# tky823/DNN-based_source_separation

Measured on AMD Instinct MI355X. Metric: separated audio frames/sec (fwd+bwd), Conv-TasNet 2-spk 4s@8kHz, higher is better.
Workload: dtype f32 (f16x3: fp32 operands/accumulators, products from a 2-part fp16 split on the fp16 MFMA; fp32-MFMA pass beside it); 1 GPU; Conv-TasNet paper-best (N=512,L=16,B=128,H=512,Sc=128,P=3,X=8,R=3) 2-spk, 4 s @ 8 kHz synthetic mixtures, 16 utterances/GPU, fwd + PIT(NegSI-SDR) + bwd + clip(5) + Adam; global_batch=16, per_gpu_batch=16, parallelism=dp1, rccl_ranks=0, launch=recorded sequence, one sep_run_sequence call per step

## Files before the change

dnn-based_source_separation_amd/csrc/gemm_coop.hip:

```cpp
#include "gemm_common.hpp"
#include <stddef.h>
#include <stdlib.h>
#include <type_traits>


namespace {

#ifndef COOP_PIPE
#define COOP_PIPE true
#endif
constexpr int CBN = 64;
constexpr int RBI = 264;
constexpr int COMAXK = 512;

template <int MI, int NS, bool AUX>
struct __attribute__((aligned(16))) CoopSmem {
    double red[8];
    float Bs[NS][4 * RBI];
    float Cs[AUX ? NS : 1][AUX ? 4 * RBI : 4];
    float Bp[2][CBN * 16];
    int be[2][CBN];
    float sc[COMAXK];
    float sh[AUX ? 4 : COMAXK];
    float epi_pad[(4 * EPI_WAVE_FLOATS > NS * 4 * RBI + (AUX ? NS * 4 * RBI : 4) + 2 * CBN * 16 + 2 * CBN + COMAXK + (AUX ? 4 : COMAXK))
                      ? 4 * EPI_WAVE_FLOATS - (NS * 4 * RBI + (AUX ? NS * 4 * RBI : 4) + 2 * CBN * 16 + 2 * CBN + COMAXK + (AUX ? 4 : COMAXK)) : 4];
};

template <int MI, int NS, bool BWD>
constexpr int coop_occupancy() {
    constexpr int by_lds = (int)((160 * 1024) / ((sizeof(CoopSmem<MI, NS, BWD>) + 511) / 512 * 512));
    constexpr int by_regs = MI == 4 ? 2 : MI == 2 ? 3 : 4;
    return by_lds < by_regs ? by_lds : by_regs;
}

__device__ __forceinline__ float co_vmax(const float a, const float b) {
    float r;
    asm("v_max_f32 %0, %1, %2" : "=v"(r) : "v"(a), "v"(b));
    return r;
}
__device__ __forceinline__ float co_quad_max(const float m) {
    float r, t;
    asm("s_nop 1\n\tv_max_f32_dpp %0, %1, %1 quad_perm:[1,0,3,2] row_mask:0xf bank_mask:0xf" : "=&v"(t) : "v"(m));
    asm("s_nop 1\n\tv_max_f32_dpp %0, %1, %1 quad_perm:[2,3,0,1] row_mask:0xf bank_mask:0xf" : "=&v"(r) : "v"(t));
    return r;
}
__device__ __forceinline__ void co_split2_pair(const float x0, const float x1, unsigned& hi, unsigned& lo) {
    const fp16x2_t h = __builtin_amdgcn_cvt_pkrtz(x0, x1);
    hi = __builtin_bit_cast(unsigned, h);
    float l0, l1;
    asm("v_fma_mix_f32 %0, %1, 1.0, -%2 op_sel_hi:[0,0,1]" : "=v"(l0) : "v"(x0), "v"(hi));
    asm("v_fma_mix_f32 %0, %1, 1.0, -%2 op_sel:[0,0,1] op_sel_hi:[0,0,1]" : "=v"(l1) : "v"(x1), "v"(hi));
    lo = __builtin_bit_cast(unsigned, __builtin_amdgcn_cvt_pkrtz(l0, l1));
}
template <int N, int I = 0, class F>
__device__ __forceinline__ void pco_unroll(F&& f) {
    if constexpr (I < N) { f(std::integral_constant<int, I>{}); pco_unroll<N, I + 1>(f); }
}
__device__ __forceinline__ f32x16 mfma_f16(const u32x4_t a, const u32x4_t b, const f32x16 c) {
    return __builtin_amdgcn_mfma_f32_32x32x16_f16(__builtin_bit_cast(f16x8_t, a), __builtin_bit_cast(f16x8_t, b), c, 0, 0, 0);
}
__device__ __forceinline__ float quad_max(float x) {
    x = fmaxf(x, __builtin_bit_cast(float, __builtin_amdgcn_update_dpp(0, __builtin_bit_cast(int, x), 0xB1, 0xF, 0xF, true)));
    x = fmaxf(x, __builtin_bit_cast(float, __builtin_amdgcn_update_dpp(0, __builtin_bit_cast(int, x), 0x4E, 0xF, 0xF, true)));
    return x;
}
template <int N>
__device__ __forceinline__ void wait_vm_lgkm0_barrier() {
    asm volatile("" ::: "memory");
    __builtin_amdgcn_s_waitcnt(0x0070 | (N & 15) | ((N >> 4) << 14));
    __builtin_amdgcn_s_barrier();
    asm volatile("" ::: "memory");
}

template <int MI, int PRO, bool SPLIT, int EF, int NS>
__global__ __launch_bounds__(256, (coop_occupancy<MI, NS, PRO == SEP_PRO_GLN_BWD>()))
void pw_gemm_coop_kernel(const sep_gemm_desc d) {
    constexpr bool P_PRELU = PRO == SEP_PRO_PRELU || PRO == SEP_PRO_GLN_PRELU;
    constexpr bool P_GLN = PRO == SEP_PRO_GLN || PRO == SEP_PRO_GLN_PRELU;
    constexpr bool P_BWD = PRO == SEP_PRO_GLN_BWD;
    constexpr int RW = 32 * MI;
    constexpr int BMc = 4 * RW;
    __shared__ CoopSmem<MI, NS, P_BWD> sm;
    using CoSmem = CoopSmem<MI, NS, P_BWD>;
    static_assert(sizeof(CoSmem) - offsetof(CoSmem, Bs) >= 4 * EPI_WAVE_FLOATS * sizeof(float), "epilogue transpose buffer");
    const int tid = threadIdx.x, lane = tid & 63;
    const int wid = __builtin_amdgcn_readfirstlane(tid >> 6);
    const int lk = lane >> 5, l31 = lane & 31;

    const int NR = d.M / BMc;
    const int ntile_t = d.ldt / CBN;
    const int NC = d.B * ntile_t;
    const int bid = blockIdx.x;
    const int xcd = bid & 7, jj = bid >> 3;
    const int rt = jj % NR;
    const int ct = (jj / NR) * 8 + xcd;
    if (ct >= NC) return;
    const int b = ct / ntile_t;
    const int t0 = (ct % ntile_t) * CBN;
    const int m0 = rt * BMc;
    const int nk = d.K / DK;
    const bool dead_tile = !P_BWD && t0 >= d.T;

    float alpha_p = 0.f, mu = 0.f, rstd = 1.f, mg = 0.f, mgx = 0.f;
    if (P_PRELU || P_BWD) alpha_p = d.pro_alpha[0];
    if (P_GLN || P_BWD) {
        gln_mu_rstd(d.pro_stats + (size_t)b * SEP_STATS_SLOTS * 2, d.count, d.eps, mu, rstd);
        for (int k = tid; k < d.K; k += 256) {
            if (P_BWD) sm.sc[k] = d.pro_gamma[k];
            else {
                const float scv = d.pro_gamma[k] * rstd;
                sm.sc[k] = scv;
                sm.sh[k] = d.pro_beta[k] - mu * scv;
            }
        }
    }
    if (P_BWD) {
        if (d.pro_bacc) gln_bwd_means(d.pro_bacc + (size_t)b * SEP_STATS_SLOTS * 2, d.pro_stats + (size_t)b * SEP_STATS_SLOTS * 2, d.count, d.eps, mg, mgx);
        else { mg = d.pro_bsum[2 * b]; mgx = d.pro_bsum[2 * b + 1]; }
    }
    float dalpha_pro = 0.f;
    asm volatile("" :: "v"(alpha_p), "v"(mu), "v"(rstd), "v"(mg), "v"(mgx));

    const int Ks1 = SPLIT ? d.k_split : d.K;
    const int split_chunk = SPLIT ? d.k_split / DK : -1;
    const size_t stepX = (size_t)DK * d.ldt;
    const unsigned offX = 4u * (unsigned)((lane >> 4) * d.ldt + 4 * (lane & 15));
    const float* baseX = d.X + ((size_t)b * Ks1 + 4 * wid) * d.ldt + t0;
    const float* baseC = P_BWD ? d.pro_aux + ((size_t)b * Ks1 + 4 * wid) * d.ldt + t0 : nullptr;
    int xi = 0, xst = 0;
    auto issue_x = [&]() {
        if (SPLIT && xi == split_chunk) baseX = d.X2 + ((size_t)b * (d.K - d.k_split) + 4 * wid) * d.ldt + t0;
        glds16_asm_once(baseX, offX, lds_addr(&sm.Bs[xst][wid * RBI]));
        if (P_BWD) glds16_asm_once(baseC, offX, lds_addr(&sm.Cs[P_BWD ? xst : 0][wid * RBI]));
        baseX += stepX;
        if (P_BWD) baseC += stepX;
        ++xi;
        xst = xst + 1 == NS ? 0 : xst + 1;
    };
    const char* Apk = reinterpret_cast<const char*>(d.A_pk) + (size_t)((m0 + wid * RW) >> 5) * nk * 2048;
    const unsigned a_lane = 16u * (unsigned)lane;

    f32x16 acc[MI][2];
#pragma unroll
    for (int mi = 0; mi < MI; ++mi)
#pragma unroll
        for (int ni = 0; ni < 2; ++ni)
#pragma unroll
            for (int r = 0; r < 16; ++r) acc[mi][ni][r] = 0.f;

    const int fsw = (l31 >> 2) & 3;
    const int c_hi = l31 * 16 + 4 * ((2 * lk) ^ fsw);
    const int c_lo = l31 * 16 + 4 * ((2 * lk + 1) ^ fsw);
    int bcur[2] = {0, 0};

    const int kq = lane & 3;
    const int col_s = 16 * wid + (lane >> 2);
    const int s_raw = kq * RBI + col_s;
    const int s_fsw = (col_s >> 2) & 3;
    const int s_hi = col_s * 16 + 4 * ((2 * (kq >> 1)) ^ s_fsw) + 2 * (kq & 1);
    const int s_lo = col_s * 16 + 4 * ((2 * (kq >> 1) + 1) ^ s_fsw) + 2 * (kq & 1);
    const bool s_live = t0 + col_s < d.T;
    const unsigned st_lane_off = 4u * (unsigned)(4 * kq * d.ldt + col_s);
    constexpr int UNSET = 10000;
    int bexp = UNSET;
    const bool fast_prelu = alpha_p >= 0.f && alpha_p <= 1.f;

    float raw[4], aux[4], v[4];
    float4 sc4 = make_float4(0.f, 0.f, 0.f, 0.f), sh4 = sc4;
    auto read_raw = [&](const int stage, const int kn) {
        const float* Bb = sm.Bs[stage];
#pragma unroll
        for (int j = 0; j < 4; ++j) raw[j] = Bb[s_raw + j * 64];
        if (P_BWD) {
            const float* Cb = sm.Cs[P_BWD ? stage : 0];
#pragma unroll
            for (int j = 0; j < 4; ++j) aux[j] = Cb[s_raw + j * 64];
        }
        if (P_GLN || P_BWD) sc4 = ld4(&sm.sc[kn * DK + 4 * kq]);
        if (P_GLN) sh4 = ld4(&sm.sh[kn * DK + 4 * kq]);
    };
    auto pro_vals = [&](const int kn) {
        const float scv[4] = {sc4.x, sc4.y, sc4.z, sc4.w};
        const float shv[4] = {sh4.x, sh4.y, sh4.z, sh4.w};
#pragma unroll
        for (int j = 0; j < 4; ++j) {
            float x = raw[j];
            if (P_BWD) {
                const float a = aux[j];
                const float u = prelu_f(a, alpha_p);
                const float xh = (u - mu) * rstd;
                const float du = rstd * (scv[j] * x - mg - xh * mgx);
                const float da = s_live ? du * prelu_grad(a, alpha_p) : 0.f;
                if (rt == 0) {
                    if (s_live && a <= 0.f) dalpha_pro += du * a;
                    float* srow = d.pro_store + ((size_t)b * d.K + kn * DK + j) * d.ldt + t0;
                    *reinterpret_cast<float*>(reinterpret_cast<char*>(srow) + (size_t)st_lane_off) = da;
                }
                x = da;
            } else {
                if (P_PRELU) x = fast_prelu ? co_vmax(x, alpha_p * x) : prelu_f(x, alpha_p);
                if (P_GLN) x = fmaf(x, scv[j], shv[j]);
            }
            v[j] = x;
        }
    };
    auto scale_vals = [&]() {
        float m = fmaxf(fmaxf(fabsf(v[0]), fabsf(v[1])), fmaxf(fabsf(v[2]), fabsf(v[3])));
        m = co_quad_max(m);
        const int e = __builtin_amdgcn_frexp_expf(m);
        const int e2 = __builtin_bit_cast(int, m) == 0 ? -3 * UNSET : e;
        bexp = e2 + bexp > 14 ? 9 - e : bexp;
    };
    unsigned h01, l01, h23, l23;
    auto split_vals = [&]() {
#pragma unroll
        for (int j = 0; j < 4; ++j) v[j] = __builtin_ldexpf(v[j], bexp);
        co_split2_pair(v[0], v[1], h01, l01);
        co_split2_pair(v[2], v[3], h23, l23);
    };
    auto write_vals = [&](const int pb) {
        float* Bp = sm.Bp[pb];
        *reinterpret_cast<uint2*>(Bp + s_hi) = make_uint2(h01, h23);
        *reinterpret_cast<uint2*>(Bp + s_lo) = make_uint2(l01, l23);
        sm.be[pb][col_s] = bexp;
    };

    u32x4_t pa[2][MI][2], pbv[2][2];
    int en[2];
    auto load_a = [&](auto setc, const int chunk) {
        constexpr int q = decltype(setc)::value;
#pragma unroll
        for (int mi = 0; mi < MI; ++mi) {
            const char* src = Apk + ((size_t)mi * nk + chunk) * 2048;
            pa[q][mi][0] = *reinterpret_cast<const u32x4_t*>(src + a_lane);
            pa[q][mi][1] = *reinterpret_cast<const u32x4_t*>(src + 1024 + a_lane);
        }
    };
    auto read_b = [&](const int pb) {
        const float* Bp = sm.Bp[pb];
#pragma unroll
        for (int ni = 0; ni < 2; ++ni) {
            pbv[ni][0] = *reinterpret_cast<const u32x4_t*>(Bp + ni * 32 * 16 + c_hi);
            pbv[ni][1] = *reinterpret_cast<const u32x4_t*>(Bp + ni * 32 * 16 + c_lo);
            en[ni] = sm.be[pb][ni * 32 + l31];
        }
    };
    auto rescale = [&]() {
#pragma unroll
        for (int ni = 0; ni < 2; ++ni) {
            const int delta = en[ni] - bcur[ni];
            if (__builtin_amdgcn_ballot_w64(delta != 0) != 0) {
#pragma unroll
                for (int mi = 0; mi < MI; ++mi)
#pragma unroll
                    for (int r = 0; r < 16; ++r) acc[mi][ni][r] = __builtin_ldexpf(acc[mi][ni][r], delta);
            }
            bcur[ni] = en[ni];
        }
    };
    constexpr int NM = 6 * MI;
    auto M = [&](auto setc, auto ic) {
        constexpr int q = decltype(setc)::value, i = decltype(ic)::value;
        constexpr int part = i / (2 * MI), mi = (i % (2 * MI)) / 2, ni = i % 2;
        constexpr int asel = part == 1 ? 1 : 0, bsel = part == 0 ? 1 : 0;
        acc[mi][ni] = mfma_f16(pa[q][mi][asel], pbv[ni][bsel], acc[mi][ni]);
        __builtin_amdgcn_sched_barrier(0);
    };
#define CO_I(k) std::integral_constant<int, (k)>{}
#define CO_SB() __builtin_amdgcn_sched_barrier(0)
    constexpr int GX = P_BWD ? 2 : 1;
    constexpr int KEEP = P_BWD ? 0 : (NS - 2) * GX + 2 * MI;
    static_assert(KEEP < 64, "vmcnt field");
    auto step = [&](auto pc, const int s) {
        constexpr int P = decltype(pc)::value;
        const bool more = s + 1 < nk;
        read_b(s & 1);
        if (more) {
            read_raw((s + 1) % NS, s + 1);
            load_a(CO_I(P ^ 1), s + 1);
        }
        CO_SB();
        rescale();
        CO_SB();
        pco_unroll<NM / 3>([&](auto ic) { M(CO_I(P), ic); });
        if (more) pro_vals(s + 1);
        CO_SB();
        pco_unroll<NM / 6>([&](auto ic) { M(CO_I(P), CO_I(decltype(ic)::value + NM / 3)); });
        if (more) scale_vals();
        CO_SB();
        pco_unroll<NM / 6>([&](auto ic) { M(CO_I(P), CO_I(decltype(ic)::value + NM / 2)); });
        if (more) split_vals();
        CO_SB();
        pco_unroll<NM / 6>([&](auto ic) { M(CO_I(P), CO_I(decltype(ic)::value + 2 * NM / 3)); });
        if (more) write_vals((s + 1) & 1);
        CO_SB();
        pco_unroll<NM / 6>([&](auto ic) { M(CO_I(P), CO_I(decltype(ic)::value + 5 * NM / 6)); });
        if (more) {
            if (KEEP > 0 && s + NS < nk) wait_vm_lgkm0_barrier<KEEP>();
            else wait_vm_lgkm0_barrier<0>();
            if (xi < nk) issue_x();
        }
    };

    if (!dead_tile) {
        __syncthreads();
        issue_x();
#pragma unroll
        for (int g = 0; g < NS - 1; ++g)
            if (xi < nk) issue_x();
        load_a(CO_I(0), 0);
        wait_vm_lgkm0_barrier<0>();
        read_raw(0, 0);
        pro_vals(0);
        scale_vals();
        split_vals();
        write_vals(0);
        wait_vm_lgkm0_barrier<0>();
        if (xi < nk) issue_x();
        int s = 0;
        for (; s + 1 < nk; s += 2) {
            step(CO_I(0), s);
            step(CO_I(1), s + 1);
        }
        if (s < nk) step(CO_I(0), s);
#pragma unroll
        for (int mi = 0; mi < MI; ++mi)
#pragma unroll
            for (int ni = 0; ni < 2; ++ni)
#pragma unroll
                for (int r = 0; r < 16; ++r) acc[mi][ni][r] = __builtin_ldexpf(acc[mi][ni][r], -bcur[ni]);
    }
    __syncthreads();
    int etid = tid, eb = b, em0 = m0, et0 = t0;
    asm volatile("" : "+v"(etid), "+s"(eb), "+s"(em0), "+s"(et0));
    const int ewid = __builtin_amdgcn_readfirstlane(etid >> 6);
    const int elane = etid & 63;
    gemm_epilogue<EF, MI, true, 4, COOP_PIPE>(d, acc, eb, em0, et0, ewid, 0, elane >> 5, elane & 31, etid, &sm.Bs[0][0], sm.red, CBN);
    if (P_BWD && rt == 0) {
        const double sdal = block_sum_256<double>((double)dalpha_pro, sm.red);
        if (tid == 0) atomicAdd(d.pro_dalpha, sdal);
    }
}

constexpr int PMAXSEG = 64;
struct PackArgs {
    sep_pack_seg seg[PMAXSEG];
    int blk_start[PMAXSEG + 1];
    int nseg;
};

__global__ __launch_bounds__(256) void pack_weights_kernel(const PackArgs a) {
    int sgi = 0;
    while (sgi + 1 < a.nseg && (int)blockIdx.x >= a.blk_start[sgi + 1]) ++sgi;
    const sep_pack_seg sg = a.seg[sgi];
    const int lane = threadIdx.x & 63;
    const int m = ((int)blockIdx.x - a.blk_start[sgi]) * 4 + (threadIdx.x >> 6);
    if (m >= sg.M) return;
    const int ng = sg.K / 8;
    float amax = 0.f;
    for (int g = lane; g < ng; g += 64) {
#pragma unroll
        for (int e = 0; e < 8; ++e) {
            const int k = 8 * g + e;
            const float x = sg.trans ? sg.W[(size_t)k * sg.ldw + m] : sg.W[(size_t)m * sg.ldw + k];
            amax = fmaxf(amax, fabsf(x));
        }
    }
#pragma unroll
    for (int o = 32; o > 0; o >>= 1) amax = fmaxf(amax, __shfl_xor(amax, o, 64));
    const int aexp = 13 - __builtin_amdgcn_frexp_expf(amax);
    if (lane == 0) sg.rscale[m] = __builtin_ldexpf(1.f, -aexp);
    uint4* dst = reinterpret_cast<uint4*>(sg.dst) + (size_t)(m >> 5) * (ng >> 1) * 128 + (m & 31);
    for (int g = lane; g < ng; g += 64) {
        float x[8];
#pragma unroll
        for (int e = 0; e < 8; ++e) {
            const int k = 8 * g + e;
            x[e] = __builtin_ldexpf(sg.trans ? sg.W[(size_t)k * sg.ldw + m] : sg.W[(size_t)m * sg.ldw + k], aexp);
        }
        unsigned hi[4], lo[4];
#pragma unroll
        for (int q = 0; q < 4; ++q) split2_pair(x[2 * q], x[2 * q + 1], hi[q], lo[q]);
        uint4* q = dst + (size_t)(g >> 1) * 128 + 32 * (g & 1);
        q[0] = make_uint4(hi[0], hi[1], hi[2], hi[3]);
        q[64] = make_uint4(lo[0], lo[1], lo[2], lo[3]);
    }
}

template <int MI, int PRO, bool SPLIT, int EF>
void launch_coop(const sep_gemm_desc& d, const int ns, hipStream_t stream) {
    const int NR = d.M / (128 * MI);
    const int NC = d.B * (d.ldt / CBN);
    const int grid = 8 * NR * ceil_div(NC, 8);
    if (ns == 3) hipLaunchKernelGGL((pw_gemm_coop_kernel<MI, PRO, SPLIT, EF, 3>), dim3(grid), dim3(256), 0, stream, d);
    else hipLaunchKernelGGL((pw_gemm_coop_kernel<MI, PRO, SPLIT, EF, 2>), dim3(grid), dim3(256), 0, stream, d);
}

}

#ifndef SEP_COOP_MI4_DEFAULT
#define SEP_COOP_MI4_DEFAULT 2
#endif
int sep_pw_gemm_packed(const sep_gemm_desc* d, hipStream_t stream) {
    static const bool off = getenv("SEPK_COOP") != nullptr && atoi(getenv("SEPK_COOP")) == 0;
    static const char* kern = getenv("SEPK_GEMM_KERNEL");
    static const bool only_coop = kern != nullptr && kern[0] == 'c';
    static const bool all_pc = kern != nullptr && kern[0] == 'p';
    static const int pc_min_k = getenv("SEPK_PC_MINK") ? atoi(getenv("SEPK_PC_MINK")) : 512;
    static const int force_mi = getenv("SEPK_COOP_MI") ? atoi(getenv("SEPK_COOP_MI")) : 0;
    static const int env_ns = getenv("SEPK_COOP_NS") ? atoi(getenv("SEPK_COOP_NS")) : 0;
    if (off || !d->A_pk || !d->a_rscale || d->arith != SEP_ARITH_F16X3) return 0;
    if (!only_coop && (all_pc || d->K >= pc_min_k || d->M >= 1024) && sep_pw_gemm_pc(d, stream)) return 1;
    if (d->M % 128 != 0 || d->K % DK != 0 || d->k_split % DK != 0 || (d->m_split % 128) != 0) return 0;
    if (d->pro_mode >= SEP_PRO_GLN && d->K > COMAXK) return 0;
    if ((size_t)d->M * d->K * 4 >= (1ull << 32) || (size_t)4 * d->ldt * 4 >= (1ull << 31)) return 0;
    const int ef = d->epi_flags, pm = d->pro_mode;
    const bool sp = d->k_split != 0;
    const int mi = (force_mi == 1 || d->M % 256 != 0) ? 1 : 2;
    const int ns = env_ns == 2 || env_ns == 3 ? env_ns : 2;
    static const int mi4 = force_mi == 4 ? 7 : getenv("SEPK_COOP_MI4") ? atoi(getenv("SEPK_COOP_MI4")) : SEP_COOP_MI4_DEFAULT;
    if ((mi4 & 1) && force_mi != 1 && force_mi != 2 && d->M % 512 == 0 && !sp && pm == SEP_PRO_NONE && ef == SEP_EPI_STATS_PRELU) { launch_coop<4, SEP_PRO_NONE, false, SEP_EPI_STATS_PRELU>(*d, ns, stream); return 1; }
    if ((mi4 & 2) && force_mi != 1 && force_mi != 2 && d->M % 512 == 0 && sp && pm == SEP_PRO_NONE && ef == 0) { launch_coop<4, SEP_PRO_NONE, true, 0>(*d, ns, stream); return 1; }
    if ((mi4 & 4) && force_mi != 1 && force_mi != 2 && d->M % 512 == 0 && !sp && pm == SEP_PRO_NONE && ef == 0) { launch_coop<4, SEP_PRO_NONE, false, 0>(*d, ns, stream); return 1; }
#define SEP_LC(P, S, E)                                              \
    do {                                                             \
        if (mi == 2) launch_coop<2, P, S, E>(*d, ns, stream);        \
        else launch_coop<1, P, S, E>(*d, ns, stream);                \
        return 1;                                                    \
    } while (0)
    if (!sp && pm == SEP_PRO_NONE && ef == SEP_EPI_STATS_PRELU) SEP_LC(SEP_PRO_NONE, false, SEP_EPI_STATS_PRELU);
    if (!sp && pm == SEP_PRO_GLN_PRELU && ef == SEP_EPI_RESIDUAL) SEP_LC(SEP_PRO_GLN_PRELU, false, SEP_EPI_RESIDUAL);
    if (!sp && pm == SEP_PRO_GLN_PRELU && ef == 0) SEP_LC(SEP_PRO_GLN_PRELU, false, 0);
    if (!sp && pm == SEP_PRO_PRELU && ef == SEP_EPI_SIGMOID) SEP_LC(SEP_PRO_PRELU, false, SEP_EPI_SIGMOID);
    if (!sp && pm == SEP_PRO_PRELU && ef == 0) SEP_LC(SEP_PRO_PRELU, false, 0);
    if (!sp && pm == SEP_PRO_GLN && ef == 0) SEP_LC(SEP_PRO_GLN, false, 0);
    if (!sp && pm == SEP_PRO_NONE && ef == 0) SEP_LC(SEP_PRO_NONE, false, 0);
    if (!sp && pm == SEP_PRO_NONE && ef == SEP_EPI_PRELU_BWD) SEP_LC(SEP_PRO_NONE, false, SEP_EPI_PRELU_BWD);
    if (sp && pm == SEP_PRO_NONE && ef == 0) SEP_LC(SEP_PRO_NONE, true, 0);
    if (sp && pm == SEP_PRO_NONE && ef == (SEP_EPI_ROWSUMS | SEP_EPI_ROWSUMS_PRELU)) SEP_LC(SEP_PRO_NONE, true, SEP_EPI_ROWSUMS | SEP_EPI_ROWSUMS_PRELU);
    if (!sp && pm == SEP_PRO_NONE && ef == (SEP_EPI_ROWSUMS | SEP_EPI_ROWSUMS_PRELU)) SEP_LC(SEP_PRO_NONE, false, SEP_EPI_ROWSUMS | SEP_EPI_ROWSUMS_PRELU);
    if (!sp && pm == SEP_PRO_NONE && ef == SEP_EPI_ROWSUMS) SEP_LC(SEP_PRO_NONE, false, SEP_EPI_ROWSUMS);
    if (!sp && pm == SEP_PRO_GLN_BWD && ef == SEP_EPI_RESIDUAL) SEP_LC(SEP_PRO_GLN_BWD, false, SEP_EPI_RESIDUAL);
    if (!sp && pm == SEP_PRO_GLN_BWD && ef == 0) SEP_LC(SEP_PRO_GLN_BWD, false, 0);
#undef SEP_LC
    return 0;
}

extern "C" int sep_pack_weights(const sep_pack_seg* segs, int nseg, sep_stream_t stream) {
    SEP_REQUIRE(segs && nseg >= 1, "sep_pack_weights: no segments");
    for (int s0 = 0; s0 < nseg; s0 += PMAXSEG) {
        PackArgs a;
        const int n = nseg - s0 < PMAXSEG ? nseg - s0 : PMAXSEG;
        int blocks = 0;
        for (int i = 0; i < n; ++i) {
            const sep_pack_seg& s = segs[s0 + i];
            SEP_REQUIRE(s.W && s.dst && s.rscale && s.M > 0 && s.K > 0 && s.K % 16 == 0 && s.M % 32 == 0 && s.ldw > 0, "sep_pack_weights: bad segment %d (M=%d K=%d)", s0 + i, s.M, s.K);
            SEP_REQUIRE((reinterpret_cast<size_t>(s.dst) & 31) == 0, "sep_pack_weights: dst of segment %d is not 32-byte aligned", s0 + i);
            a.seg[i] = s;
            a.blk_start[i] = blocks;
            blocks += ceil_div(s.M, 4);
        }
        a.blk_start[n] = blocks;
        a.nseg = n;
        hipLaunchKernelGGL(pack_weights_kernel, dim3(blocks), dim3(256), 0, (hipStream_t)stream, a);
        SEP_CHECK_LAUNCH("sep_pack_weights");
    }
    return 0;
}
```

Before: 4.291 million frames/s.

## Rewrite weight packing kernel with coalesced shared-memory tiles per 32 rows

The weight pack kernel now handles 32 output rows per block. It stages 128-wide K chunks through a padded shared-memory tile using float4 coalesced loads, with a register prefetch of the next chunk, instead of one wave per row doing strided scalar reads (badly strided in the transposed case). Segment lookup becomes a binary search over a slimmer structure-of-arrays argument block, so up to 112 segments fit in one launch. The cost is extra shared memory, barriers and a two-pass read of W for the amax.

```diff
diff --git a/dnn-based_source_separation_amd/csrc/gemm_coop.hip b/dnn-based_source_separation_amd/csrc/gemm_coop.hip
--- a/dnn-based_source_separation_amd/csrc/gemm_coop.hip
+++ b/dnn-based_source_separation_amd/csrc/gemm_coop.hip
@@ -342,48 +342,112 @@
     }
 }
 
-constexpr int PMAXSEG = 64;
+constexpr int PMAXSEG = 112;
+constexpr int PKC = 128;
 struct PackArgs {
-    sep_pack_seg seg[PMAXSEG];
+    const float* W[PMAXSEG];
+    void* dst[PMAXSEG];
+    float* rscale[PMAXSEG];
+    int kt[PMAXSEG];
+    int ldw[PMAXSEG];
     int blk_start[PMAXSEG + 1];
     int nseg;
 };
+static_assert(sizeof(PackArgs) <= 4096, "kernel arguments");
 
 __global__ __launch_bounds__(256) void pack_weights_kernel(const PackArgs a) {
-    int sgi = 0;
-    while (sgi + 1 < a.nseg && (int)blockIdx.x >= a.blk_start[sgi + 1]) ++sgi;
-    const sep_pack_seg sg = a.seg[sgi];
-    const int lane = threadIdx.x & 63;
-    const int m = ((int)blockIdx.x - a.blk_start[sgi]) * 4 + (threadIdx.x >> 6);
-    if (m >= sg.M) return;
-    const int ng = sg.K / 8;
-    float amax = 0.f;
-    for (int g = lane; g < ng; g += 64) {
-#pragma unroll
-        for (int e = 0; e < 8; ++e) {
-            const int k = 8 * g + e;
-            const float x = sg.trans ? sg.W[(size_t)k * sg.ldw + m] : sg.W[(size_t)m * sg.ldw + k];
-            amax = fmaxf(amax, fabsf(x));
-        }
-    }
-#pragma unroll
-    for (int o = 32; o > 0; o >>= 1) amax = fmaxf(amax, __shfl_xor(amax, o, 64));
-    const int aexp = 13 - __builtin_amdgcn_frexp_expf(amax);
-    if (lane == 0) sg.rscale[m] = __builtin_ldexpf(1.f, -aexp);
-    uint4* dst = reinterpret_cast<uint4*>(sg.dst) + (size_t)(m >> 5) * (ng >> 1) * 128 + (m & 31);
-    for (int g = lane; g < ng; g += 64) {
-        float x[8];
-#pragma unroll
-        for (int e = 0; e < 8; ++e) {
-            const int k = 8 * g + e;
-            x[e] = __builtin_ldexpf(sg.trans ? sg.W[(size_t)k * sg.ldw + m] : sg.W[(size_t)m * sg.ldw + k], aexp);
-        }
-        unsigned hi[4], lo[4];
-#pragma unroll
-        for (int q = 0; q < 4; ++q) split2_pair(x[2 * q], x[2 * q + 1], hi[q], lo[q]);
-        uint4* q = dst + (size_t)(g >> 1) * 128 + 32 * (g & 1);
-        q[0] = make_uint4(hi[0], hi[1], hi[2], hi[3]);
-        q[64] = make_uint4(lo[0], lo[1], lo[2], lo[3]);
+    __shared__ float tile[32][PKC + 1];
+    __shared__ unsigned s_amax[32];
+    int sgi = 0, sgh = a.nseg - 1;
+    while (sgi < sgh) {
+        const int mid = (sgi + sgh + 1) >> 1;
+        if ((int)blockIdx.x >= a.blk_start[mid]) sgi = mid;
+        else sgh = mid - 1;
+    }
+    const float* __restrict__ W = a.W[sgi];
+    const int K = a.kt[sgi] & ~1, ldw = a.ldw[sgi];
+    const bool trans = (a.kt[sgi] & 1) != 0;
+    const int m0 = 32 * ((int)blockIdx.x - a.blk_start[sgi]);
+    const int t = threadIdx.x, lane = t & 63, row = lane & 31;
+    const bool vec = (reinterpret_cast<size_t>(W) & 15) == 0 && (ldw & 3) == 0;
+    auto fetch = [&](const int idx, const int k0, bool& ok) -> float4 {
+        const int kk = trans ? idx >> 3 : 4 * (idx & 31);
+        const int r = trans ? 4 * (idx & 7) : idx >> 5;
+        ok = k0 + kk < K;
+        if (!ok) return make_float4(0.f, 0.f, 0.f, 0.f);
+        const float* p = trans ? W + (size_t)(k0 + kk) * ldw + m0 + r : W + (size_t)(m0 + r) * ldw + k0 + kk;
+        if (vec) return *reinterpret_cast<const float4*>(p);
+        return make_float4(p[0], p[1], p[2], p[3]);
+    };
+    if (t < 32) s_amax[t] = 0u;
+    __syncthreads();
+    float am[4] = {0.f, 0.f, 0.f, 0.f};
+    for (int k0 = 0; k0 < K; k0 += PKC) {
+#pragma unroll
+        for (int i = 0; i < 4; ++i) {
+            bool ok;
+            const float4 v = fetch(t + 256 * i, k0, ok);
+            if (trans) {
+                am[0] = fmaxf(am[0], fabsf(v.x));
+                am[1] = fmaxf(am[1], fabsf(v.y));
+                am[2] = fmaxf(am[2], fabsf(v.z));
+                am[3] = fmaxf(am[3], fabsf(v.w));
+            } else {
+                am[i] = fmaxf(fmaxf(fmaxf(am[i], fabsf(v.x)), fabsf(v.y)), fmaxf(fabsf(v.z), fabsf(v.w)));
+            }
+        }
+    }
+#pragma unroll
+    for (int i = 0; i < 4; ++i) {
+        if (trans) {
+#pragma unroll
+            for (int o = 8; o < 64; o <<= 1) am[i] = fmaxf(am[i], __shfl_xor(am[i], o, 64));
+            if (lane < 8) atomicMax(&s_amax[4 * lane + i], __float_as_uint(am[i]));
+        } else {
+#pragma unroll
+            for (int o = 1; o < 32; o <<= 1) am[i] = fmaxf(am[i], __shfl_xor(am[i], o, 64));
+            if (row == 0) atomicMax(&s_amax[(t >> 5) + 8 * i], __float_as_uint(am[i]));
+        }
+    }
+    __syncthreads();
+    const int aexp = 13 - __builtin_amdgcn_frexp_expf(__uint_as_float(s_amax[row]));
+    if (t < 32) a.rscale[sgi][m0 + t] = __builtin_ldexpf(1.f, -aexp);
+    uint4* dst = reinterpret_cast<uint4*>(a.dst[sgi]) + (size_t)(m0 >> 5) * (K >> 4) * 128 + lane;
+    float4 v[4];
+    bool ok[4];
+#pragma unroll
+    for (int i = 0; i < 4; ++i) v[i] = fetch(t + 256 * i, 0, ok[i]);
+    for (int k0 = 0; k0 < K; k0 += PKC) {
+#pragma unroll
+        for (int i = 0; i < 4; ++i) {
+            const int idx = t + 256 * i;
+            if (!ok[i]) continue;
+            if (trans) {
+                const int kk = idx >> 3, r = 4 * (idx & 7);
+                tile[r][kk] = v[i].x, tile[r + 1][kk] = v[i].y, tile[r + 2][kk] = v[i].z, tile[r + 3][kk] = v[i].w;
+            } else {
+                const int kk = 4 * (idx & 31), r = idx >> 5;
+                tile[r][kk] = v[i].x, tile[r][kk + 1] = v[i].y, tile[r][kk + 2] = v[i].z, tile[r][kk + 3] = v[i].w;
+            }
+        }
+        __syncthreads();
+        if (k0 + PKC < K) {
+#pragma unroll
+            for (int i = 0; i < 4; ++i) v[i] = fetch(t + 256 * i, k0 + PKC, ok[i]);
+        }
+        for (int c = t >> 6; c < PKC / 16 && k0 + 16 * c < K; c += 4) {
+            const float* src = &tile[row][16 * c + 8 * (lane >> 5)];
+            float x[8];
+#pragma unroll
+            for (int e = 0; e < 8; ++e) x[e] = __builtin_ldexpf(src[e], aexp);
+            unsigned hi[4], lo[4];
+#pragma unroll
+            for (int q = 0; q < 4; ++q) split2_pair(x[2 * q], x[2 * q + 1], hi[q], lo[q]);
+            uint4* q = dst + (size_t)((k0 >> 4) + c) * 128;
+            q[0] = make_uint4(hi[0], hi[1], hi[2], hi[3]);
+            q[64] = make_uint4(lo[0], lo[1], lo[2], lo[3]);
+        }
+        __syncthreads();
     }
 }
 
@@ -456,9 +520,11 @@
             const sep_pack_seg& s = segs[s0 + i];
             SEP_REQUIRE(s.W && s.dst && s.rscale && s.M > 0 && s.K > 0 && s.K % 16 == 0 && s.M % 32 == 0 && s.ldw > 0, "sep_pack_weights: bad segment %d (M=%d K=%d)", s0 + i, s.M, s.K);
             SEP_REQUIRE((reinterpret_cast<size_t>(s.dst) & 31) == 0, "sep_pack_weights: dst of segment %d is not 32-byte aligned", s0 + i);
-            a.seg[i] = s;
+            a.W[i] = s.W, a.dst[i] = s.dst, a.rscale[i] = s.rscale;
+            a.kt[i] = s.K | (s.trans ? 1 : 0);
+            a.ldw[i] = s.ldw;
             a.blk_start[i] = blocks;
-            blocks += ceil_div(s.M, 4);
+            blocks += s.M / 32;
         }
         a.blk_start[n] = blocks;
         a.nseg = n;
```

After: 4.307 million frames/s, median of 6. About the same (+0.4%).
